# matthewyjiang/safe_bayesian_optimization

Hardware: AMD Instinct MI355X
Metric: GP posterior+acq grid-points/sec at N train pts; 1/2/4/8 GPU (higher is better)
Workload: dtype f32 (bf16x3-split MFMA, f32 accumulation)

## Files before the change

safe_bayesian_optimization_amd/csrc/diag/predict_x3_diag.hip:

```cpp
#include <cstdint>
#include <cstdlib>
#include <algorithm>
#include <type_traits>
#include <vector>

#include "../sbo_internal.hpp"

namespace sbo {
namespace {

typedef float f32x4 __attribute__((ext_vector_type(4)));
typedef float f32x2 __attribute__((ext_vector_type(2)));
typedef __bf16 bf16x2 __attribute__((ext_vector_type(2)));
typedef __bf16 bf16x8 __attribute__((ext_vector_type(8)));
typedef unsigned int u32x4 __attribute__((ext_vector_type(4)));

constexpr int kXH = 32;
constexpr int kXPlane = kBM * kXH * 2;
constexpr int kXA = 3 * kXPlane;
constexpr int kXC = 4 * kXH * 4;
constexpr int kXQ = 2 * kBN * 4;
constexpr int kXSlot = kXA + kXC + kXQ;
constexpr int kXSlots = 3;
constexpr int kXWin = kXSlots * kXSlot;
// ... 422 lines not shown
            }                                                                                           \
            if (lane < 32) SBO_DMA16(kc3 + (uint32_t)(kcf_) + (h_) * (kXC / 4), d_ + kXA);              \
        }                                                                                               \
        const char *s_ = a_base + ((DIAG & 8) ? 0 : (uint64_t)((akib_) + (h_) * (kXA / 1024)) * 1024u);  \
        const uint32_t w_ = lds_wave + (uint32_t)(sl_) * kXSlot;                                        \
        a_src = s_;                                                                                     \
        a_dst = w_;                                                                                     \
        if (!(DIAG & 2) && is_loader && ((burst_) || !(DIAG & 16)))                                     \
            _Pragma("unroll") for (int j = 0; j < kPieces; ++j)                                         \
                SBO_DMA16(s_ + j * kLoaders * 1024, w_ + (uint32_t)(j * kLoaders * 1024));              \
    } while (0)
#define SBO_REC_WINDOW(w_)                                                                              \
    do {                                                                                                \
        if (lw == 1) SBO_DMA16(reinterpret_cast<const char *>(rec) + (uint64_t)(w_) * 1024u, lds_rwin + (uint32_t)((w_) & 1) * 1024u); \
    } while (0)
    auto rec_at = [&](uint32_t e) {
        const int4 d = rwin[((e / kRecWin) & 1) * kRecWin + e % kRecWin];
        return make_int4(__builtin_amdgcn_readfirstlane(d.x), __builtin_amdgcn_readfirstlane(d.y),
                         __builtin_amdgcn_readfirstlane(d.z), __builtin_amdgcn_readfirstlane(d.w));
    };
    uint32_t la_e, e_end;
    {
        const int4 da = desc[k0], db = desc[k1 - 1];
        la_e = (uint32_t)__builtin_amdgcn_readfirstlane(da.z);
        e_end = (uint32_t)__builtin_amdgcn_readfirstlane(db.z) + (uint32_t)(__builtin_amdgcn_readfirstlane(db.w) & 0xffff);
    }
    SBO_REC_WINDOW(la_e / kRecWin);
    SBO_REC_WINDOW(la_e / kRecWin + 1);
    asm volatile("s_waitcnt vmcnt(0)" ::: "memory");
    __syncthreads();
    int la_h = 0;

    const char *a_base = ax3 + (is_loader ? ldr : 0) * 1024;
    const char *a_src = ax3;
    uint32_t a_dst = 0;
    int4 r_cur = rec_at(la_e);
    auto stage = [&](int sl, bool burst) {
        const int4 r = r_cur;
        XStep s;
        s.I = min(r.w & 0xffff, nI - 1);
        s.qb = r.z;
        s.flags = la_h | ((r.w & kRecFirst) && la_h == 0 ? kFirst : 0) | ((r.w & kRecLast) && la_h == 1 ? kLast : 0) |
                  kValid;
        s.lv = LEVELS ? min((r.w >> 16) & 3, 2) : 0;
        SBO_X3_STAGE(min((uint32_t)r.x, a_max), r.y, la_h, r.z, sl, burst, (s.flags & kFirst) != 0);
        la_h ^= 1;
        if (la_h == 0) {
            ++la_e;
            if (la_e % kRecWin == 1) SBO_REC_WINDOW(la_e / kRecWin + 1);
            if (la_e < e_end) r_cur = rec_at(la_e);
        }
        return s;
    };

    XStep s0 = stage(0, true), s1 = {0, 0, 0, 0}, s2 = {0, 0, 0, 0};
    if (la_e < e_end) s1 = stage(1, true);
    asm volatile("s_waitcnt vmcnt(0)" ::: "memory");
    __syncthreads();

    const int qo = WIDE ? lw * 32 + (lane & 31) : lw * 16 * NC + r;
    constexpr int kCB = NC == 2 ? 2 : 1, kRB = WIDE ? 8 : 16;
    typedef std::conditional_t<WIDE, f32x16, f32x4> AccT;
    AccT acc[kCB][kRB], outer[kCB][kRB];
#pragma unroll
    for (int c = 0; c < kCB; ++c)
#pragma unroll
// ... 274 lines not shown
            const double v = (double)h[sl * kStampFields + j];
            if (j < n) out[j] += v;
            const int o = 12 + 12 * (int)(sl % 8) + j;
            if (o < n) out[o] += v;
        }
        const int o = 108 + (int)(sl / 8);
        if (o < n) out[o] += (double)h[sl * kStampFields + 5] / 8.0;
    }
    std::fill(h.begin(), h.end(), 0ull);
    return hipMemcpyToSymbol(HIP_SYMBOL(g_x3_stamps), h.data(), h.size() * sizeof(unsigned long long));
}

hipError_t launch_predict_x3(hipStream_t s, const char *ax3, const float *kc3, const int4 *desc, const int4 *rec,
                             const int *seg, int P, int n_items, int nI, const float *qx, const float *qy, int64_t m,
                             int64_t ldp, float cexp, float m0, float *part, float *mean, int variant) {
    const int64_t amax = (total_tiles(nI) - 1) * (2 * kXA / 1024);
    if (nI <= 0 || amax > 0xffffffffll) return hipErrorInvalidValue;
    const uint32_t a_max = (uint32_t)amax;
    int rot = 0;
#ifdef SBO_DIAG
    if (const char *e = getenv("SBO_XCD_ROT")) rot = std::clamp(atoi(e), 0, 7);
#endif
#define SBO_X3_LAUNCH(NC, D) \
    hipLaunchKernelGGL((predict_x3_kernel<NC, D>), dim3((unsigned)P), dim3(NC == 1 ? 512 : 256), 0, s, ax3, kc3, desc, rec, \
                       seg, P, n_items, nI, a_max, rot, qx, qy, m, ldp, cexp, m0, part, mean)
    switch (variant) {
        case 2: SBO_X3_LAUNCH(2, 16); break;
        case 9: SBO_X3_LAUNCH(1, 0); break;
        case 10: SBO_X3_LAUNCH(1, 48); break;
        case 13: SBO_X3_LAUNCH(3, 16); break;
        case 22: SBO_X3_LAUNCH(1, 16); break;
// ... 60 lines not shown
```

safe_bayesian_optimization_amd/csrc/kernels.hip:

```cpp
#include <cstdio>
#include <cstdlib>
#include <algorithm>
#include <cstring>

#include <rocprim/rocprim.hpp>

#include "sbo_internal.hpp"

namespace sbo {
namespace {

typedef float f32x16 __attribute__((ext_vector_type(16)));

__device__ __forceinline__ float fast_exp2(float v) { return __builtin_amdgcn_exp2f(v); }

constexpr int kFillCols = 8;

template <bool VEC>
__global__ __launch_bounds__(256) void rbf_fill_kernel(const float *__restrict__ xa,
                                                       const float *__restrict__ ya, int64_t ma,
                                                       const float *__restrict__ xb,
                                                       const float *__restrict__ yb, int64_t mb,
                                                       int64_t ld, float c, float sf2, float sn2,
                                                       int diag, float *__restrict__ K) {
// ... 1876 lines not shown
    const int64_t a = xseg[x], n = xseg[x + 1] - a, q = n / G, rm = n % G, c = (k - a) % G, j = (k - a) / G;
    return a + c * q + (c < rm ? c : rm) + j;
}

__global__ void plan_perm_kernel(const unsigned long long *__restrict__ scan, int64_t n_items,
                                 const int4 *__restrict__ desc, const int *__restrict__ xseg, int G,
                                 int *__restrict__ pos_of, unsigned long long *__restrict__ cnt2) {
    const int64_t nne = (int64_t)(scan[n_items - 1] >> kPlanKeyShift);
    const int64_t k = (int64_t)blockIdx.x * blockDim.x + threadIdx.x;
    if (k >= nne) return;
    const int64_t p = xcd_position(k, xseg, G);
    pos_of[k] = (int)p;
    cnt2[p] = (unsigned long long)(desc[k].w & 0xffff);
}

__device__ __forceinline__ int4 step_record(int64_t ts, int I, int qb, int te, int i, int cnt);

__global__ __launch_bounds__(256) void plan_move_kernel(const unsigned long long *__restrict__ scan, int64_t n_items,
                                                        const int4 *__restrict__ desc,
                                                        const unsigned short *__restrict__ tl,
                                                        const int *__restrict__ pos_of,
                                                        const unsigned long long *__restrict__ off2,
                                                        int4 *__restrict__ desc2, unsigned short *__restrict__ tl2,
                                                        int4 *__restrict__ rec) {
    const int64_t nne = (int64_t)(scan[n_items - 1] >> kPlanKeyShift);
    const int64_t k = (int64_t)blockIdx.x * 4 + (threadIdx.x >> 6);
    const int lane = threadIdx.x & 63;
    if (k >= nne) return;
    const int4 d = desc[k];
    const int cnt = d.w & 0xffff;
    const uint64_t off = (uint64_t)(uint32_t)d.z | ((uint64_t)((uint32_t)d.w >> 16) << 32);
    const int p = pos_of[k];
    const uint64_t o2 = off2[p];
    const int64_t ts = tile_start(d.x);
    for (int i = lane; i < cnt; i += 64) {
        const unsigned short te = tl[off + i];
        tl2[o2 + i] = te;
        if (rec) rec[o2 + i] = step_record(ts, d.x, d.y, te, i, cnt);
    }
    if (lane == 0) desc2[p] = make_int4(d.x, d.y, (int)(uint32_t)o2, cnt | (int)((o2 >> 32) << 16));
}

__device__ __forceinline__ int4 step_record(int64_t ts, int I, int qb, int te, int i, int cnt) {
    const int t = te & ((1 << kLevelShift) - 1);
    const int w = I | ((te >> kLevelShift) << 16) | (i == 0 ? kRecFirst : 0) | (i == cnt - 1 ? kRecLast : 0);
    return make_int4((int)(uint32_t)((ts + t) * 96), t * 256, qb, w);
}

__global__ __launch_bounds__(256) void plan_rec_kernel(const unsigned long long *__restrict__ scan, int64_t n_items,
                                                       const int4 *__restrict__ desc,
                                                       const unsigned short *__restrict__ tl, int4 *__restrict__ rec) {
    const int64_t nne = (int64_t)(scan[n_items - 1] >> kPlanKeyShift);
    const int64_t k = (int64_t)blockIdx.x * 4 + (threadIdx.x >> 6);
    const int lane = threadIdx.x & 63;
    if (k >= nne) return;
    const int4 d = desc[k];
    const int cnt = d.w & 0xffff;
    const uint64_t off = (uint64_t)(uint32_t)d.z | ((uint64_t)((uint32_t)d.w >> 16) << 32);
    const int64_t ts = tile_start(d.x);
    for (int i = lane; i < cnt; i += 64) rec[off + i] = step_record(ts, d.x, d.y, tl[off + i], i, cnt);
}

__global__ void plan_seg2_kernel(const int *__restrict__ xseg, int G, int P, int *__restrict__ seg2) {
    for (int r = threadIdx.x; r <= P; r += blockDim.x) {
        if (r == P) {
            seg2[P] = xseg[8];
            continue;
        }
        const int x = r / G, c = r % G;
        const int a = xseg[x], n = xseg[x + 1] - a, q = n / G, rm = n % G;
        seg2[r] = a + c * q + (c < rm ? c : rm);
    }
}

__global__ void plan_block_cost_kernel(const unsigned long long *__restrict__ wkey, int nI, int64_t nQ,
// ... 534 lines not shown
    auto take = [&](size_t b) {
        const size_t at = o;
        o = (o + b + 255) / 256 * 256;
        return at;
    };
    L.key = take(8 * (size_t)items);
    L.scan = take(8 * (size_t)items);
    L.thr = take((size_t)items);
    L.wkey = take(8 * (size_t)items);
    L.wscan = take(8 * (size_t)items);
    L.lvcnt = take(8 * 3 * 4 * (size_t)kPlanWriteBlocks);
    L.bits = take(8 * 3 * (size_t)items * (size_t)plan_chunks((int)nI));
    L.desc = take(16 * (size_t)(items + 2 * kDescWindow));
    L.tl = take(2 * (size_t)(cap + 2 * kListWindow));
    L.seg = take(4 * (size_t)(P + 1));
    L.rec = take(16 * (size_t)(cap + 2 * kRecWindow));
    size_t tb = 0;
    (void)rocprim::inclusive_scan(nullptr, tb, (const unsigned long long *)nullptr, (unsigned long long *)nullptr,
                                  (size_t)items, rocprim::plus<unsigned long long>());
    L.temp = take(tb);
    L.temp_bytes = tb;
    L.xcd = xcd_interleave(P);
    if (L.xcd) {
        L.xseg = take(4 * 9);
        L.pos_of = take(4 * (size_t)items);
        L.cnt2 = take(8 * (size_t)items);
        L.off2 = take(8 * (size_t)items);
        L.desc2 = take(16 * (size_t)(items + 2 * kDescWindow));
        L.tl2 = take(2 * (size_t)(cap + 2 * kListWindow));
        L.seg2 = take(4 * (size_t)(P + 1));
        size_t t2 = 0;
// ... 12 lines not shown

size_t predict_work_bytes(int64_t npad, int64_t m, int P) {
    return plan_layout(npad / kBM, (m + kBN - 1) / kBN, P).total;
}

hipError_t launch_plan(hipStream_t s, const float4 *kbox, int64_t npad, const float *qx, const float *qy, int64_t m,
                       int64_t ldp, float ell, float m0, const SkipPlan &skip, float *part, float *mean,
                       unsigned long long *tiles_done, int P, void *work, size_t work_bytes) {
    const int nI = (int)(npad / kBM);
    const int64_t nQ = (m + kBN - 1) / kBN;
    const int64_t items = (int64_t)nI * nQ;
    if (m <= 0 || nI <= 0) return hipSuccess;
    if (nQ > 0x7fffffff || items >= (1ll << (64 - kPlanKeyShift)) ||
        2 * (int64_t)nI * (nI + 1) * nQ >= (1ll << kPlanKeyShift) || kTilesPerRowBlockStep * (int64_t)nI > (1 << kLevelShift) - 1)
        return hipErrorInvalidValue;
    const PlanLayout L = plan_layout(nI, nQ, P);
    if (work_bytes < L.total) return hipErrorInvalidValue;
    if (skip.order_blk != 0 && ((skip.order_blk >> 8) < 1 || (skip.order_blk & 255) < 1 || (skip.order_blk >> 16) != 0))
        return hipErrorInvalidValue;
    char *w = static_cast<char *>(work);
    auto *key = reinterpret_cast<unsigned long long *>(w + L.key);
    auto *scan = reinterpret_cast<unsigned long long *>(w + L.scan);
    auto *thr = reinterpret_cast<unsigned char *>(w + L.thr);
    auto *desc = reinterpret_cast<int4 *>(w + L.desc);
    auto *tl = reinterpret_cast<unsigned short *>(w + L.tl);
    auto *seg = reinterpret_cast<int *>(w + L.seg);
    auto *wkey = reinterpret_cast<unsigned long long *>(w + L.wkey);
    auto *wscan = reinterpret_cast<unsigned long long *>(w + L.wscan);
#ifdef SBO_DIAG
    if (const char *ev = getenv("SBO_MEAN_W")) {
// ... 29 lines not shown
    e = rocprim::inclusive_scan(w + L.temp, tb, wkey, wscan, (size_t)items, rocprim::plus<unsigned long long>(), s);
    if (e != hipSuccess) return e;
    const int64_t wblocks = std::min<int64_t>((items + 3) / 4, kPlanWriteBlocks);
    hipLaunchKernelGGL(plan_write_kernel, dim3((unsigned)wblocks), dim3(256), 0, s, nI, nQ, key, scan, bits,
                       desc, tl, skip.prod_full, tiles_done ? reinterpret_cast<unsigned long long *>(w + L.lvcnt) : nullptr,
                       skip.order_blk);
    if (tiles_done)
        hipLaunchKernelGGL(plan_counts_reduce_kernel, dim3(1), dim3(256), 0, s,
                           reinterpret_cast<const unsigned long long *>(w + L.lvcnt), wblocks * 4, tiles_done + 1);
    auto *rec = reinterpret_cast<int4 *>(w + L.rec);
    if (!L.xcd) {
        hipLaunchKernelGGL(plan_seg_kernel, dim3(1), dim3(256), 0, s, scan, items, desc, P, seg, tiles_done, wkey,
                           wscan, nI, nQ, skip.order_blk);
        if (skip.records)
            hipLaunchKernelGGL(plan_rec_kernel, dim3((unsigned)((items + 3) / 4)), dim3(256), 0, s, scan, items, desc,
                               tl, rec);
        return hipGetLastError();
    }
    auto *xseg = reinterpret_cast<int *>(w + L.xseg);
    auto *pos_of = reinterpret_cast<int *>(w + L.pos_of);
    auto *cnt2 = reinterpret_cast<unsigned long long *>(w + L.cnt2);
    auto *off2 = reinterpret_cast<unsigned long long *>(w + L.off2);
    auto *desc2 = reinterpret_cast<int4 *>(w + L.desc2);
    auto *tl2 = reinterpret_cast<unsigned short *>(w + L.tl2);
    auto *seg2 = reinterpret_cast<int *>(w + L.seg2);
    const int G = P / 8;
    e = hipMemsetAsync(cnt2, 0, 8 * (size_t)items, s);
    if (e != hipSuccess) return e;
    hipLaunchKernelGGL(plan_seg_kernel, dim3(1), dim3(256), 0, s, scan, items, desc, 8, xseg, tiles_done, wkey, wscan,
                       nI, nQ, skip.order_blk);
    hipLaunchKernelGGL(plan_perm_kernel, dim3((unsigned)((items + 255) / 256)), dim3(256), 0, s, scan, items, desc,
                       xseg, G, pos_of, cnt2);
    e = hipGetLastError();
    if (e != hipSuccess) return e;
    size_t t2 = L.temp2_bytes;
    e = rocprim::exclusive_scan(w + L.temp2, t2, cnt2, off2, 0ull, (size_t)items,
                                rocprim::plus<unsigned long long>(), s);
    if (e != hipSuccess) return e;
    hipLaunchKernelGGL(plan_move_kernel, dim3((unsigned)((items + 3) / 4)), dim3(256), 0, s, scan, items, desc, tl,
                       pos_of, off2, desc2, tl2, skip.records ? rec : nullptr);
    hipLaunchKernelGGL(plan_seg2_kernel, dim3(1), dim3(256), 0, s, xseg, G, P, seg2);
    return hipGetLastError();
}

void plan_views(int64_t npad, int64_t m, int P, const void *work, const int4 **desc, const unsigned short **tl,
                const int **seg, const int4 **rec) {
    const PlanLayout L = plan_layout(npad / kBM, (m + kBN - 1) / kBN, P);
    const char *w = static_cast<const char *>(work);
    *desc = reinterpret_cast<const int4 *>(w + (L.xcd ? L.desc2 : L.desc));
    *tl = reinterpret_cast<const unsigned short *>(w + (L.xcd ? L.tl2 : L.tl));
    *seg = reinterpret_cast<const int *>(w + (L.xcd ? L.seg2 : L.seg));
    if (rec) *rec = reinterpret_cast<const int4 *>(w + L.rec);
}

float exp2_coef_f(float ell) { return (float)exp2_coef(ell); }
// ... 82 lines not shown
```

safe_bayesian_optimization_amd/csrc/predict_x3.hip:

```cpp
#include <cstdint>
#include <vector>

#include "sbo_internal.hpp"

namespace sbo {
namespace {

typedef float f32x4 __attribute__((ext_vector_type(4)));
typedef float f32x2 __attribute__((ext_vector_type(2)));
typedef __bf16 bf16x2 __attribute__((ext_vector_type(2)));
typedef __bf16 bf16x8 __attribute__((ext_vector_type(8)));
typedef unsigned int u32x4 __attribute__((ext_vector_type(4)));

constexpr int kXH = 32;
constexpr int kXPlane = kBM * kXH * 2;
constexpr int kXA = 3 * kXPlane;
constexpr int kXC = 4 * kXH * 4;
constexpr int kXQ = 2 * kBN * 4;
constexpr int kXSlot = kXA + kXC + kXQ;
constexpr int kXSlots = 3;
constexpr int kXWin = kXSlots * kXSlot;
constexpr int kXSmem = kXWin + 4096;
constexpr int kRecWin = 64;
constexpr int kLoaders = 8;
// ... 16 lines not shown
    w1 = pk_bf16(ra, rb);
    w2 = pk_bf16(ra - lo_f32(w1), rb - hi_f32(w1));
}

__device__ __forceinline__ bf16x8 as_bf16x8(u32x4 v) { return __builtin_bit_cast(bf16x8, v); }

__device__ __forceinline__ f32x4 mfma(u32x4 a, u32x4 b, f32x4 c) {
    return __builtin_amdgcn_mfma_f32_16x16x32_bf16(as_bf16x8(a), as_bf16x8(b), c, 0, 0, 0);
}

typedef __attribute__((address_space(3))) char lds_char;

__device__ __forceinline__ u32x4 lds_b128(const lds_char *p) {
    return *reinterpret_cast<const __attribute__((address_space(3))) u32x4 *>(p);
}
__device__ __forceinline__ float lds_f(const lds_char *p) {
    return *reinterpret_cast<const __attribute__((address_space(3))) float *>(p);
}
typedef float f32x2v __attribute__((ext_vector_type(2)));
__device__ __forceinline__ f32x2v lds_f2(const lds_char *p) {
    return *reinterpret_cast<const __attribute__((address_space(3))) f32x2v *>(p);
}

__device__ __forceinline__ void dma16_masked(uint32_t voff, const void *sbase, uint32_t ldst, uint64_t mask) {
    uint64_t sv;
    asm volatile("s_mov_b64 %0, exec\n\ts_and_b64 exec, exec, %4\n\ts_nop 0\n\tglobal_load_lds_dwordx4 %1, %2\n\t"
                 "s_mov_b64 exec, %0"
                 : "=&s"(sv)
                 : "v"(voff), "s"(sbase), "{m0}"(ldst), "s"(mask)
                 : "memory", "scc");
}

struct KPieces {
    u32x4 h, m, l;
};

__device__ __forceinline__ float kstar1(float xk, float yk, float xq, float yq, float cexp) {
    const float dx = xk - xq, dy = yk - yq;
    return fast_exp2(fmaf(dy, dy, dx * dx) * cexp);
}

#define SBO_PIN(v) asm volatile("" : "+v"(v))

template <bool FRESH, int LV, bool KHN>
__device__ __forceinline__ void x3_half(const lds_char *pa, const lds_char *pcn, float xq, float yq, int g,
                                        float cexp, float msc, const KPieces &kb, f32x4 (&acc)[16],
                                        f32x4 (&outer)[16], KPieces &nx, double &mu, uint32_t voff, const char *asrc,
                                        uint32_t adst, int npieces) {
    const f32x4 zero = {0.f, 0.f, 0.f, 0.f};
    constexpr bool P1 = LV <= 1, P2 = LV == 0;
    constexpr int NPROD = LV == 0 ? 6 : (LV == 1 ? 3 : 1);
    constexpr int LAG = LV == 0 ? 2 : (LV == 1 ? 4 : 8);
    constexpr int AH = LV == 2 ? 4 : (LV == 1 ? 2 : 1);
    u32x4 f0[16], f1[16], f2[16];
#pragma unroll
    for (int r = 0; r < AH; ++r) {
        f0[r] = lds_b128(pa + r * 1024);
        if constexpr (P1) f1[r] = lds_b128(pa + kXPlane + r * 1024);
        if constexpr (P2) f2[r] = lds_b128(pa + 2 * kXPlane + r * 1024);
    }
    f32x2v xk = lds_f2(pcn + g * 32), yk = lds_f2(pcn + 128 + g * 32), ak = {0.f, 0.f};
    if (msc != 0.0f) ak = lds_f2(pcn + 256 + g * 32);
    f32x2v e;
#pragma unroll
    for (int rb = 0; rb < 16; ++rb) {
        if (rb + AH < 16) {
            f0[rb + AH] = lds_b128(pa + (rb + AH) * 1024);
            if constexpr (P1) f1[rb + AH] = lds_b128(pa + kXPlane + (rb + AH) * 1024);
            if constexpr (P2) f2[rb + AH] = lds_b128(pa + 2 * kXPlane + (rb + AH) * 1024);
        }
        const u32x4 a0 = f0[rb];
        u32x4 a1 = {}, a2 = {};
        if constexpr (P1) a1 = f1[rb];
        if constexpr (P2) a2 = f2[rb];
        const int i = rb >> 2, ph = rb & 3;
        if (ph <= 1) {
            float ev = kstar1(ph == 0 ? xk.x : xk.y, ph == 0 ? yk.x : yk.y, xq, yq, cexp);
            SBO_PIN(ev);
            if (ph == 0) e.x = ev; else e.y = ev;
            if (ph == 1 && i < 3) {
// ... 11 lines not shown
                SBO_PIN(w0);
                SBO_PIN(w1);
                SBO_PIN(w2);
                nx.h[i] = w0;
                nx.m[i] = w1;
                nx.l[i] = w2;
            }
        } else {
            if (msc != 0.0f) {
                mu += (double)fmaf(ak.x, e.x, ak.y * e.y);
                SBO_PIN(mu);
            }
            if (i < 3 && msc != 0.0f) ak = lds_f2(pcn + 256 + g * 32 + (i + 1) * 8);
        }
        if (rb >= 1 && rb <= kPieces) {
            const uint32_t mh = (uint32_t)__builtin_amdgcn_readfirstlane(rb <= npieces ? -1 : 0);
            dma16_masked(voff, asrc + (rb - 1) * kStride, adst + (rb - 1) * kStride, ((uint64_t)mh << 32) | mh);
        }
        if (!FRESH && rb >= LAG) outer[rb - LAG] += acc[rb - LAG];
        f32x4 v = FRESH ? zero : acc[rb];
        if constexpr (P2) {
            v = mfma(a2, kb.h, v);
            v = mfma(a1, kb.m, v);
            v = mfma(a0, kb.l, v);
        }
        if constexpr (P1) {
            v = mfma(a1, kb.h, v);
            v = mfma(a0, kb.m, v);
        }
        v = mfma(a0, kb.h, v);
        acc[rb] = v;
#pragma unroll
        for (int j = 0; j < NPROD; ++j) {
            __builtin_amdgcn_sched_group_barrier(0x008, 1, 0);
            __builtin_amdgcn_sched_group_barrier(0x002, 2, 0);
            __builtin_amdgcn_sched_group_barrier(0x100, 1, 0);
        }
        __builtin_amdgcn_sched_barrier(0);
    }
    if (!FRESH) {
#pragma unroll
        for (int rb = 16 - LAG; rb < 16; ++rb) outer[rb] += acc[rb];
    }
}

__device__ __forceinline__ void x3_kstar(const lds_char *pc, float xq, float yq, int g, float cexp, bool mean,
                                         KPieces &kb, double &mu) {
#pragma unroll
    for (int i = 0; i < 4; ++i) {
        const f32x2v xk = lds_f2(pc + g * 32 + i * 8), yk = lds_f2(pc + 128 + g * 32 + i * 8);
        const f32x2v ak = lds_f2(pc + 256 + g * 32 + i * 8);
        const float e0 = kstar1(xk.x, yk.x, xq, yq, cexp), e1 = kstar1(xk.y, yk.y, xq, yq, cexp);
        uint32_t w0, w1, w2;
        split3(e0, e1, w0, w1, w2);
        kb.h[i] = w0;
        kb.m[i] = w1;
        kb.l[i] = w2;
        if (mean) mu += (double)fmaf(ak.x, e0, ak.y * e1);
    }
}

struct XStep {
    int I, qb, flags;
    int lv;
};
constexpr int kFirst = 2, kLast = 4, kValid = 8;

__global__ __launch_bounds__(512, 1) void predict_x3_kernel(
    const char *__restrict__ ax3, const float *__restrict__ kc3, const int4 *__restrict__ desc,
    const int4 *__restrict__ rec, const int *__restrict__ seg, int P, int n_items, int nI, uint32_t a_max,
    const float *__restrict__ qx, const float *__restrict__ qy, int64_t m, int64_t ldp, float cexp, float m0,
    float *__restrict__ part, float *__restrict__ mean) {
    __shared__ __attribute__((aligned(16))) char smem[kXSmem];
    const int bid = blockIdx.x;
    const int rng = (P % 8 == 0) ? (bid % 8) * (P / 8) + bid / 8 : bid;
    const int k0 = max(seg[rng], 0), k1 = min(seg[rng + 1], n_items);
    if (k0 >= k1) return;
    const int tid = threadIdx.x, lane = tid & 63;
    const int lw = __builtin_amdgcn_readfirstlane(tid >> 6);
    const int g = lane >> 4, r = lane & 15;

    const lds_char *lds = (const lds_char *)smem;
    const int4 *rwin = reinterpret_cast<const int4 *>(smem + kXWin);
    const uint32_t voff = (uint32_t)lane * 16u;
    const uint32_t lds_smem = (uint32_t)(uintptr_t)(lds_char *)(smem);
    const uint32_t lds_wave = lds_smem + (uint32_t)lw * 1024u;
    const uint32_t lds_rwin = lds_smem + (uint32_t)kXWin;
#define SBO_DMA16(sbase, ldst)                                                                          \
    asm volatile("s_nop 0\n\tglobal_load_lds_dwordx4 %0, %1" ::"v"(voff), "s"((const void *)(sbase)),     \
                 "{m0}"(ldst)                                                                           \
                 : "memory")
#define SBO_X3_STAGE(akib_, kcf_, h_, qb_, sl_, burst_, first_)                                         \
    do {                                                                                                \
        const uint32_t d_ = lds_smem + (uint32_t)(sl_) * kXSlot;                                        \
        if (lw == 0) {                                                                                  \
            if (first_) {                                                                               \
                if (lane < 32) SBO_DMA16(qx + (int64_t)(qb_) * kBN, d_ + kXA + kXC);                    \
                else SBO_DMA16(qy + (int64_t)(qb_) * kBN - 128, d_ + kXA + kXC);                        \
            }                                                                                           \
            if (lane < 32) SBO_DMA16(kc3 + (uint32_t)(kcf_) + (h_) * (kXC / 4), d_ + kXA);              \
        }                                                                                               \
        const char *s_ = a_base + (uint64_t)((akib_) + (h_) * (kXA / 1024)) * 1024u;                     \
        const uint32_t w_ = lds_wave + (uint32_t)(sl_) * kXSlot;                                        \
        a_src = s_;                                                                                     \
        a_dst = w_;                                                                                     \
        if (burst_)                                                                                     \
            _Pragma("unroll") for (int j = 0; j < kPieces; ++j)                                         \
                SBO_DMA16(s_ + j * kStride, w_ + (uint32_t)(j * kStride));                              \
    } while (0)
#define SBO_REC_WINDOW(w_)                                                                              \
    do {                                                                                                \
        if (lw == 1) SBO_DMA16(reinterpret_cast<const char *>(rec) + (uint64_t)(w_) * 1024u, lds_rwin + (uint32_t)((w_) & 1) * 1024u); \
    } while (0)
    auto rec_at = [&](uint32_t e) {
        const int4 d = rwin[((e / kRecWin) & 1) * kRecWin + e % kRecWin];
        return make_int4(__builtin_amdgcn_readfirstlane(d.x), __builtin_amdgcn_readfirstlane(d.y),
                         __builtin_amdgcn_readfirstlane(d.z), __builtin_amdgcn_readfirstlane(d.w));
    };
    uint32_t la_e, e_end;
    {
        const int4 da = desc[k0], db = desc[k1 - 1];
        la_e = (uint32_t)__builtin_amdgcn_readfirstlane(da.z);
        e_end = (uint32_t)__builtin_amdgcn_readfirstlane(db.z) + (uint32_t)(__builtin_amdgcn_readfirstlane(db.w) & 0xffff);
    }
    SBO_REC_WINDOW(la_e / kRecWin);
    SBO_REC_WINDOW(la_e / kRecWin + 1);
    asm volatile("s_waitcnt vmcnt(0)" ::: "memory");
    __syncthreads();
    int la_h = 0;

    const char *a_base = ax3 + lw * 1024;
    const char *a_src = ax3;
    uint32_t a_dst = 0;
    int4 r_cur = rec_at(la_e);
    auto stage = [&](int sl, bool burst) {
        const int4 rr = r_cur;
        XStep s;
        s.I = min(rr.w & 0xffff, nI - 1);
        s.qb = rr.z;
        s.flags = la_h | ((rr.w & kRecFirst) && la_h == 0 ? kFirst : 0) | ((rr.w & kRecLast) && la_h == 1 ? kLast : 0) |
                  kValid;
        s.lv = min((rr.w >> 16) & 3, 2);
        SBO_X3_STAGE(min((uint32_t)rr.x, a_max), rr.y, la_h, rr.z, sl, burst, (s.flags & kFirst) != 0);
        la_h ^= 1;
        if (la_h == 0) {
            ++la_e;
            if (la_e % kRecWin == 1) SBO_REC_WINDOW(la_e / kRecWin + 1);
            if (la_e < e_end) r_cur = rec_at(la_e);
        }
        return s;
    };

    XStep s0 = stage(0, true), s1 = {0, 0, 0, 0}, s2 = {0, 0, 0, 0};
    if (la_e < e_end) s1 = stage(1, true);
    asm volatile("s_waitcnt vmcnt(0)" ::: "memory");
    __syncthreads();

    const int qo = lw * 16 + r;
    f32x4 acc[16], outer[16];
#pragma unroll
    for (int rb = 0; rb < 16; ++rb) {
        acc[rb] = f32x4{};
        outer[rb] = acc[rb];
    }
    double mu = 0.0;
    KPieces kb, nx;
    float xq, yq;
    {
        const lds_char *pq = lds + kXA + kXC;
        xq = lds_f(pq + qo * 4);
        yq = lds_f(pq + (kBN + qo) * 4);
        x3_kstar(lds + kXA, xq, yq, g, cexp, s0.I == nI - 1, kb, mu);
    }
    bool pend = false, pend_mean = false;
    float pend_s = 0.0f, pend_mu = 0.0f;
    int64_t pend_q = 0;
    int pend_I = 0;
    auto flush = [&]() {
        if (pend && lane < 16 && pend_q < m) {
            part[(int64_t)pend_I * ldp + pend_q] = pend_s;
            if (pend_mean) mean[pend_q] = pend_mu;
        }
        pend = false;
    };
    int cur = 0;
    bool more = true;
    auto half_step = [&](auto fresh_tag) {
        constexpr bool FRESH = decltype(fresh_tag)::value;
        if (FRESH) flush();
        const bool issue = la_e < e_end;
        const int nslot = cur == 0 ? 2 : cur - 1;
        s2 = issue ? stage(nslot, false) : XStep{0, 0, 0, 0};
        const int np2 = (kPieces / 3) * (3 - s2.lv);
        if (!issue) a_dst = lds_wave + (uint32_t)nslot * kXSlot;
        const int cslot = cur == 2 ? 0 : cur + 1;
        const lds_char *pa = lds + cur * kXSlot + lane * 16;
        const lds_char *pcn = lds + cslot * kXSlot + kXA;
        const lds_char *pqn = pcn + kXC;
        const bool nvalid = (s1.flags & kValid) != 0;
        const float msc = nvalid && s1.I == nI - 1 ? 1.0f : 0.0f;
        if (!FRESH) {
            if ((s0.flags & kLast) && s0.I == nI - 1) {
                double u = mu;
                u += __shfl_xor(u, 16);
                u += __shfl_xor(u, 32);
                pend_mu = (float)((double)m0 + u);
            }
            if (nvalid && (s1.flags & kFirst)) mu = 0.0;
        }
        if (nvalid && (s1.flags & kFirst)) {
            xq = lds_f(pqn + qo * 4);
            yq = lds_f(pqn + (kBN + qo) * 4);
        }
        if (s0.lv == 2 && nvalid && s1.lv == 2)
            x3_half<FRESH, 2, true>(pa, pcn, xq, yq, g, cexp, msc, kb, acc, outer, nx, mu, voff, a_src, a_dst, np2);
        else if (s0.lv == 2)
            x3_half<FRESH, 2, false>(pa, pcn, xq, yq, g, cexp, msc, kb, acc, outer, nx, mu, voff, a_src, a_dst, np2);
        else if (s0.lv == 1)
            x3_half<FRESH, 1, false>(pa, pcn, xq, yq, g, cexp, msc, kb, acc, outer, nx, mu, voff, a_src, a_dst, np2);
        else
            x3_half<FRESH, 0, false>(pa, pcn, xq, yq, g, cexp, msc, kb, acc, outer, nx, mu, voff, a_src, a_dst, np2);
        if (!FRESH && (s0.flags & kLast)) {
            pend = true;
            pend_I = s0.I;
            pend_q = (int64_t)s0.qb * kBN + qo;
            pend_mean = s0.I == nI - 1;
            double sq[4] = {};
#pragma unroll
            for (int rb = 0; rb < 16; ++rb)
#pragma unroll
                for (int e = 0; e < 4; ++e) {
                    sq[e] = fma((double)outer[rb][e], (double)outer[rb][e], sq[e]);
                    outer[rb][e] = 0.0f;
                }
            double sv = (sq[0] + sq[1]) + (sq[2] + sq[3]);
            sv += __shfl_xor(sv, 16);
            sv += __shfl_xor(sv, 32);
            pend_s = (float)sv;
        }
        asm volatile("s_waitcnt vmcnt(6)" ::: "memory");
        asm volatile("s_waitcnt lgkmcnt(0)\n\ts_barrier" ::: "memory");
        more = nvalid;
        s0 = s1;
        s1 = s2;
        kb = nx;
        cur = cslot;
    };
    do {
        half_step(std::integral_constant<bool, true>{});
        half_step(std::integral_constant<bool, false>{});
    } while (more);
    asm volatile("s_waitcnt vmcnt(0)" ::: "memory");
    flush();
#undef SBO_X3_STAGE
#undef SBO_REC_WINDOW
#undef SBO_DMA16
}

__global__ __launch_bounds__(256) void pack_x3_kernel(const float *__restrict__ aug, int64_t T0, int64_t nt,
                                                      char *__restrict__ ax3) {
    const int64_t id = (int64_t)blockIdx.x * 256 + threadIdx.x;
// ... 46 lines not shown
    }
    if (!kc3) return hipSuccess;
    const int64_t nkt = npad / kBK;
    hipLaunchKernelGGL(pack_kc3_kernel, dim3((unsigned)((nkt * 256 + 255) / 256)), dim3(256), 0, s, kcoord, nkt, kc3);
    return hipGetLastError();
}

hipError_t read_x3_stamps(double *out, int n) {
    for (int j = 0; j < n; ++j) out[j] = 0.0;
    return hipSuccess;
}

hipError_t launch_predict_x3(hipStream_t s, const char *ax3, const float *kc3, const int4 *desc, const int4 *rec,
                             const int *seg, int P, int n_items, int nI, const float *qx, const float *qy, int64_t m,
                             int64_t ldp, float cexp, float m0, float *part, float *mean, int variant) {
    const int64_t amax = (total_tiles(nI) - 1) * (2 * kXA / 1024);
    if (nI <= 0 || amax > 0xffffffffll) return hipErrorInvalidValue;
    if (variant != 3 && variant != 22) return hipErrorInvalidValue;
    hipLaunchKernelGGL(predict_x3_kernel, dim3((unsigned)P), dim3(512), 0, s, ax3, kc3, desc, rec, seg, P, n_items, nI,
                       (uint32_t)amax, qx, qy, m, ldp, cexp, m0, part, mean);
    return hipGetLastError();
}

}
```

safe_bayesian_optimization_amd/csrc/sbo_internal.hpp:

```cpp
#pragma once

#include <hip/hip_runtime.h>
#include <rocblas/rocblas.h>

#include <cstddef>
#include <cstdint>
#include <string>
#include <utility>
#include <vector>

#include "../../include/sbo.h"

namespace sbo {

constexpr int kBM = 256;
constexpr int kBN = 128;
constexpr int kBK = 64;
constexpr int kTileFloats = kBM * kBK;
constexpr int kTilesPerRowBlockStep = kBM / kBK;
constexpr int kAcqThreads = 256;
constexpr int64_t kMaxGridY = 65535;

__host__ __device__ inline int64_t round_up(int64_t v, int64_t m) { return (v + m - 1) / m * m; }

// ... 223 lines not shown
                       int64_t ldp, float ell, float m0, const SkipPlan &skip, float *part, float *mean,
                       unsigned long long *tiles_done, int P, void *work, size_t work_bytes);
hipError_t launch_predict(hipStream_t s, const float *aug, const float *kcoord, int64_t npad, const float *qx,
                          const float *qy, int64_t m, int64_t ldp, float ell, float m0, float *part, float *mean,
                          int variant, int P, const void *work);
float exp2_coef_f(float ell);
hipError_t launch_plan_cost(hipStream_t s, int64_t npad, int64_t m, int P, const void *work, const int32_t *perm,
                            float *bcost, float *cost);
void plan_views(int64_t npad, int64_t m, int P, const void *work, const int4 **desc, const unsigned short **tl,
                const int **seg, const int4 **rec = nullptr);
size_t x3_operand_bytes(int64_t npad);
size_t x3_coord_bytes(int64_t npad);
hipError_t launch_pack_x3(hipStream_t s, const float *aug, const float *kcoord, int64_t npad, int64_t I0, int wide,
                          char *ax3, float *kc3);
constexpr int kLevelShift = 14;
constexpr int kRecFirst = 1 << 20, kRecLast = 1 << 21;
inline bool x3_levels(int variant) { return variant == 3 || variant == 23 || variant == 24 || variant == 30 || variant == 32 || variant == 33 || variant == 39 || variant == 41 || variant == 42 || variant == 43 || variant == 46 || variant == 47 || variant == 48 || variant == 49 || variant == 51 || variant == 52 || variant == 53 || variant == 54 || variant == 55 || variant == 56 || variant == 57 || (variant >= 58 && variant <= 61); }
inline bool variant_allowed(int v) {
#ifdef SBO_DIAG
    return v >= 0 && v <= 61;
#else
    return v == 0 || v == 1 || v == 3 || v == 22;
#endif
}
inline int x3_layout(int variant) { return (variant == 13 || variant == 14) ? 1 : 0; }
hipError_t read_x3_stamps(double *out, int n);
hipError_t launch_predict_x3(hipStream_t s, const char *ax3, const float *kc3, const int4 *desc, const int4 *rec,
                             const int *seg, int P, int n_items, int nI, const float *qx, const float *qy, int64_t m,
                             int64_t ldp, float cexp, float m0, float *part, float *mean, int variant);
hipError_t launch_tile_norms(hipStream_t s, const float *aug, int64_t npad, int64_t I0, float4 *lgn);
hipError_t launch_pack_tile_norms(hipStream_t s, const double *Linv, int64_t ld, int64_t n, int64_t npad, int64_t I0,
// ... 110 lines not shown
```

Baseline: 42.83 million.

## Precompute per-half step records to cut scalar bookkeeping in x3 predict loop

The plan kernels now emit two records per step, one per half, with clamped row block, level, half, first/last, mean and piece-count flags and final addresses all precomputed. The predict loop just reads the next record from LDS, prefetched inside x3_half with a volatile load and readfirstlane, and rotates slot offsets instead of recomputing slot indices. This removes per-half scalar ALU work (mins, flag composition, branches) and hides the record read latency behind MFMA work. In exchange the record buffer doubles and the plan gains an extra size limit. It also adds optional register pinning of the outer accumulators and an s_cselect-based DMA mask.

```diff
diff --git a/safe_bayesian_optimization_amd/csrc/diag/predict_x3_diag.hip b/safe_bayesian_optimization_amd/csrc/diag/predict_x3_diag.hip
--- a/safe_bayesian_optimization_amd/csrc/diag/predict_x3_diag.hip
+++ b/safe_bayesian_optimization_amd/csrc/diag/predict_x3_diag.hip
@@ -460,8 +460,8 @@
     do {                                                                                                \
         if (lw == 1) SBO_DMA16(reinterpret_cast<const char *>(rec) + (uint64_t)(w_) * 1024u, lds_rwin + (uint32_t)((w_) & 1) * 1024u); \
     } while (0)
-    auto rec_at = [&](uint32_t e) {
-        const int4 d = rwin[((e / kRecWin) & 1) * kRecWin + e % kRecWin];
+    auto rec_at = [&](uint32_t j) {
+        const int4 d = rwin[j % (2 * kRecWin)];
         return make_int4(__builtin_amdgcn_readfirstlane(d.x), __builtin_amdgcn_readfirstlane(d.y),
                          __builtin_amdgcn_readfirstlane(d.z), __builtin_amdgcn_readfirstlane(d.w));
     };
@@ -471,8 +471,8 @@
         la_e = (uint32_t)__builtin_amdgcn_readfirstlane(da.z);
         e_end = (uint32_t)__builtin_amdgcn_readfirstlane(db.z) + (uint32_t)(__builtin_amdgcn_readfirstlane(db.w) & 0xffff);
     }
-    SBO_REC_WINDOW(la_e / kRecWin);
-    SBO_REC_WINDOW(la_e / kRecWin + 1);
+    SBO_REC_WINDOW(2 * la_e / kRecWin);
+    SBO_REC_WINDOW(2 * la_e / kRecWin + 1);
     asm volatile("s_waitcnt vmcnt(0)" ::: "memory");
     __syncthreads();
     int la_h = 0;
@@ -480,22 +480,20 @@
     const char *a_base = ax3 + (is_loader ? ldr : 0) * 1024;
     const char *a_src = ax3;
     uint32_t a_dst = 0;
-    int4 r_cur = rec_at(la_e);
+    int4 r_cur = rec_at(2 * la_e);
     auto stage = [&](int sl, bool burst) {
         const int4 r = r_cur;
         XStep s;
-        s.I = min(r.w & 0xffff, nI - 1);
+        s.I = r.w & 0xffff;
         s.qb = r.z;
-        s.flags = la_h | ((r.w & kRecFirst) && la_h == 0 ? kFirst : 0) | ((r.w & kRecLast) && la_h == 1 ? kLast : 0) |
-                  kValid;
-        s.lv = LEVELS ? min((r.w >> 16) & 3, 2) : 0;
-        SBO_X3_STAGE(min((uint32_t)r.x, a_max), r.y, la_h, r.z, sl, burst, (s.flags & kFirst) != 0);
+        s.flags = ((r.w & kRecHalf) ? 1 : 0) | ((r.w & kRecFirst) ? kFirst : 0) | ((r.w & kRecLast) ? kLast : 0) | kValid;
+        s.lv = LEVELS ? (r.w >> kRecLevelShift) & 3 : 0;
+        SBO_X3_STAGE(min((uint32_t)r.x, a_max), r.y, 0, r.z, sl, burst, (s.flags & kFirst) != 0);
         la_h ^= 1;
-        if (la_h == 0) {
-            ++la_e;
-            if (la_e % kRecWin == 1) SBO_REC_WINDOW(la_e / kRecWin + 1);
-            if (la_e < e_end) r_cur = rec_at(la_e);
-        }
+        if (la_h == 0) ++la_e;
+        const uint32_t j = 2 * la_e + (uint32_t)la_h;
+        if (j % kRecWin == 2) SBO_REC_WINDOW(j / kRecWin + 1);
+        if (la_e < e_end) r_cur = rec_at(j);
         return s;
     };
 
@@ -800,7 +798,7 @@
 hipError_t launch_predict_x3(hipStream_t s, const char *ax3, const float *kc3, const int4 *desc, const int4 *rec,
                              const int *seg, int P, int n_items, int nI, const float *qx, const float *qy, int64_t m,
                              int64_t ldp, float cexp, float m0, float *part, float *mean, int variant) {
-    const int64_t amax = (total_tiles(nI) - 1) * (2 * kXA / 1024);
+    const int64_t amax = (total_tiles(nI) - 1) * (2 * kXA / 1024) + kXA / 1024;
     if (nI <= 0 || amax > 0xffffffffll) return hipErrorInvalidValue;
     const uint32_t a_max = (uint32_t)amax;
     int rot = 0;
diff --git a/safe_bayesian_optimization_amd/csrc/kernels.hip b/safe_bayesian_optimization_amd/csrc/kernels.hip
--- a/safe_bayesian_optimization_amd/csrc/kernels.hip
+++ b/safe_bayesian_optimization_amd/csrc/kernels.hip
@@ -1914,7 +1914,7 @@
     cnt2[p] = (unsigned long long)(desc[k].w & 0xffff);
 }
 
-__device__ __forceinline__ int4 step_record(int64_t ts, int I, int qb, int te, int i, int cnt);
+__device__ __forceinline__ int4 step_record(int64_t ts, int I, int qb, int te, int i, int cnt, int nI, int h);
 
 __global__ __launch_bounds__(256) void plan_move_kernel(const unsigned long long *__restrict__ scan, int64_t n_items,
                                                         const int4 *__restrict__ desc,
@@ -1922,7 +1922,7 @@
                                                         const int *__restrict__ pos_of,
                                                         const unsigned long long *__restrict__ off2,
                                                         int4 *__restrict__ desc2, unsigned short *__restrict__ tl2,
-                                                        int4 *__restrict__ rec) {
+                                                        int4 *__restrict__ rec, int nI) {
     const int64_t nne = (int64_t)(scan[n_items - 1] >> kPlanKeyShift);
     const int64_t k = (int64_t)blockIdx.x * 4 + (threadIdx.x >> 6);
     const int lane = threadIdx.x & 63;
@@ -1936,20 +1936,30 @@
     for (int i = lane; i < cnt; i += 64) {
         const unsigned short te = tl[off + i];
         tl2[o2 + i] = te;
-        if (rec) rec[o2 + i] = step_record(ts, d.x, d.y, te, i, cnt);
+        if (rec) {
+            rec[2 * (o2 + i)] = step_record(ts, d.x, d.y, te, i, cnt, nI, 0);
+            rec[2 * (o2 + i) + 1] = step_record(ts, d.x, d.y, te, i, cnt, nI, 1);
+        }
     }
     if (lane == 0) desc2[p] = make_int4(d.x, d.y, (int)(uint32_t)o2, cnt | (int)((o2 >> 32) << 16));
 }
 
-__device__ __forceinline__ int4 step_record(int64_t ts, int I, int qb, int te, int i, int cnt) {
+__device__ __forceinline__ int4 step_record(int64_t ts, int I, int qb, int te, int i, int cnt, int nI, int h) {
     const int t = te & ((1 << kLevelShift) - 1);
-    const int w = I | ((te >> kLevelShift) << 16) | (i == 0 ? kRecFirst : 0) | (i == cnt - 1 ? kRecLast : 0);
-    return make_int4((int)(uint32_t)((ts + t) * 96), t * 256, qb, w);
+    const int lv = min((te >> kLevelShift) & 3, 2);
+    const int rb = min(I, nI - 1);
+    const int64_t tile = min(ts + t, tile_start(nI) - 1);
+    const int w = rb | (lv << kRecLevelShift) | (h ? kRecHalf : 0) | (i == 0 && h == 0 ? kRecFirst : 0) |
+                  (i == cnt - 1 && h == 1 ? kRecLast : 0) | (rb == nI - 1 ? kRecMean : 0) | kRecValid |
+                  ((2 * (3 - lv)) << kRecPiecesShift);
+    return make_int4((int)(uint32_t)(tile * (2 * kRecHalfKiB) + h * kRecHalfKiB),
+                     t * (2 * kRecHalfCoords) + h * kRecHalfCoords, qb, w);
 }
 
 __global__ __launch_bounds__(256) void plan_rec_kernel(const unsigned long long *__restrict__ scan, int64_t n_items,
                                                        const int4 *__restrict__ desc,
-                                                       const unsigned short *__restrict__ tl, int4 *__restrict__ rec) {
+                                                       const unsigned short *__restrict__ tl, int4 *__restrict__ rec,
+                                                       int nI) {
     const int64_t nne = (int64_t)(scan[n_items - 1] >> kPlanKeyShift);
     const int64_t k = (int64_t)blockIdx.x * 4 + (threadIdx.x >> 6);
     const int lane = threadIdx.x & 63;
@@ -1958,7 +1968,8 @@
     const int cnt = d.w & 0xffff;
     const uint64_t off = (uint64_t)(uint32_t)d.z | ((uint64_t)((uint32_t)d.w >> 16) << 32);
     const int64_t ts = tile_start(d.x);
-    for (int i = lane; i < cnt; i += 64) rec[off + i] = step_record(ts, d.x, d.y, tl[off + i], i, cnt);
+    for (int j = lane; j < 2 * cnt; j += 64)
+        rec[2 * off + j] = step_record(ts, d.x, d.y, tl[off + (j >> 1)], j >> 1, cnt, nI, j & 1);
 }
 
 __global__ void plan_seg2_kernel(const int *__restrict__ xseg, int G, int P, int *__restrict__ seg2) {
@@ -2523,7 +2534,7 @@
     L.desc = take(16 * (size_t)(items + 2 * kDescWindow));
     L.tl = take(2 * (size_t)(cap + 2 * kListWindow));
     L.seg = take(4 * (size_t)(P + 1));
-    L.rec = take(16 * (size_t)(cap + 2 * kRecWindow));
+    L.rec = take(16 * (size_t)(2 * cap + 2 * kRecWindow));
     size_t tb = 0;
     (void)rocprim::inclusive_scan(nullptr, tb, (const unsigned long long *)nullptr, (unsigned long long *)nullptr,
                                   (size_t)items, rocprim::plus<unsigned long long>());
@@ -2566,6 +2577,7 @@
     if (nQ > 0x7fffffff || items >= (1ll << (64 - kPlanKeyShift)) ||
         2 * (int64_t)nI * (nI + 1) * nQ >= (1ll << kPlanKeyShift) || kTilesPerRowBlockStep * (int64_t)nI > (1 << kLevelShift) - 1)
         return hipErrorInvalidValue;
+    if (skip.records && 2 * (int64_t)nI * (nI + 1) * nQ >= (1ll << 31)) return hipErrorInvalidValue;
     const PlanLayout L = plan_layout(nI, nQ, P);
     if (work_bytes < L.total) return hipErrorInvalidValue;
     if (skip.order_blk != 0 && ((skip.order_blk >> 8) < 1 || (skip.order_blk & 255) < 1 || (skip.order_blk >> 16) != 0))
@@ -2625,7 +2637,7 @@
                            wscan, nI, nQ, skip.order_blk);
         if (skip.records)
             hipLaunchKernelGGL(plan_rec_kernel, dim3((unsigned)((items + 3) / 4)), dim3(256), 0, s, scan, items, desc,
-                               tl, rec);
+                               tl, rec, nI);
         return hipGetLastError();
     }
     auto *xseg = reinterpret_cast<int *>(w + L.xseg);
@@ -2649,7 +2661,7 @@
                                 rocprim::plus<unsigned long long>(), s);
     if (e != hipSuccess) return e;
     hipLaunchKernelGGL(plan_move_kernel, dim3((unsigned)((items + 3) / 4)), dim3(256), 0, s, scan, items, desc, tl,
-                       pos_of, off2, desc2, tl2, skip.records ? rec : nullptr);
+                       pos_of, off2, desc2, tl2, skip.records ? rec : nullptr, nI);
     hipLaunchKernelGGL(plan_seg2_kernel, dim3(1), dim3(256), 0, s, xseg, G, P, seg2);
     return hipGetLastError();
 }
diff --git a/safe_bayesian_optimization_amd/csrc/predict_x3.hip b/safe_bayesian_optimization_amd/csrc/predict_x3.hip
--- a/safe_bayesian_optimization_amd/csrc/predict_x3.hip
+++ b/safe_bayesian_optimization_amd/csrc/predict_x3.hip
@@ -54,6 +54,9 @@
 __device__ __forceinline__ u32x4 lds_b128(const lds_char *p) {
     return *reinterpret_cast<const __attribute__((address_space(3))) u32x4 *>(p);
 }
+__device__ __forceinline__ u32x4 lds_b128_here(const lds_char *p) {
+    return *reinterpret_cast<const volatile __attribute__((address_space(3))) u32x4 *>(p);
+}
 __device__ __forceinline__ float lds_f(const lds_char *p) {
     return *reinterpret_cast<const __attribute__((address_space(3))) float *>(p);
 }
@@ -82,11 +85,15 @@
 
 #define SBO_PIN(v) asm volatile("" : "+v"(v))
 
+#ifndef SBO_X3_OUTER_PIN
+#define SBO_X3_OUTER_PIN 7
+#endif
+
 template <bool FRESH, int LV, bool KHN>
 __device__ __forceinline__ void x3_half(const lds_char *pa, const lds_char *pcn, float xq, float yq, int g,
                                         float cexp, float msc, const KPieces &kb, f32x4 (&acc)[16],
                                         f32x4 (&outer)[16], KPieces &nx, double &mu, uint32_t voff, const char *asrc,
-                                        uint32_t adst, int npieces) {
+                                        uint32_t adst, int npieces, const lds_char *prec, int4 &rnx) {
     const f32x4 zero = {0.f, 0.f, 0.f, 0.f};
     constexpr bool P1 = LV <= 1, P2 = LV == 0;
     constexpr int NPROD = LV == 0 ? 6 : (LV == 1 ? 3 : 1);
@@ -102,8 +109,11 @@
     f32x2v xk = lds_f2(pcn + g * 32), yk = lds_f2(pcn + 128 + g * 32), ak = {0.f, 0.f};
     if (msc != 0.0f) ak = lds_f2(pcn + 256 + g * 32);
     f32x2v e;
+    u32x4 rraw = {};
+    const int nps = __builtin_amdgcn_readfirstlane(npieces);
 #pragma unroll
     for (int rb = 0; rb < 16; ++rb) {
+        if (rb == 16 - AH) rraw = lds_b128_here(prec);
         if (rb + AH < 16) {
             f0[rb + AH] = lds_b128(pa + (rb + AH) * 1024);
             if constexpr (P1) f1[rb + AH] = lds_b128(pa + kXPlane + (rb + AH) * 1024);
@@ -145,10 +155,14 @@
             if (i < 3 && msc != 0.0f) ak = lds_f2(pcn + 256 + g * 32 + (i + 1) * 8);
         }
         if (rb >= 1 && rb <= kPieces) {
-            const uint32_t mh = (uint32_t)__builtin_amdgcn_readfirstlane(rb <= npieces ? -1 : 0);
-            dma16_masked(voff, asrc + (rb - 1) * kStride, adst + (rb - 1) * kStride, ((uint64_t)mh << 32) | mh);
-        }
-        if (!FRESH && rb >= LAG) outer[rb - LAG] += acc[rb - LAG];
+            uint64_t mask;
+            asm("s_cmp_ge_u32 %1, %2\n\ts_cselect_b64 %0, -1, 0" : "=s"(mask) : "s"(nps), "n"(rb) : "scc");
+            dma16_masked(voff, asrc + (rb - 1) * kStride, adst + (rb - 1) * kStride, mask);
+        }
+        if (!FRESH && rb >= LAG) {
+            outer[rb - LAG] += acc[rb - LAG];
+            if constexpr (((SBO_X3_OUTER_PIN) >> LV) & 1) SBO_PIN(outer[rb - LAG]);
+        }
         f32x4 v = FRESH ? zero : acc[rb];
         if constexpr (P2) {
             v = mfma(a2, kb.h, v);
@@ -169,6 +183,11 @@
         }
         __builtin_amdgcn_sched_barrier(0);
     }
+    rnx.x = __builtin_amdgcn_readfirstlane((int)rraw.x);
+    rnx.y = __builtin_amdgcn_readfirstlane((int)rraw.y);
+    rnx.z = __builtin_amdgcn_readfirstlane((int)rraw.z);
+    rnx.w = __builtin_amdgcn_readfirstlane((int)rraw.w);
+    asm volatile("" : "+s"(rnx.x), "+s"(rnx.y), "+s"(rnx.z), "+s"(rnx.w));
     if (!FRESH) {
 #pragma unroll
         for (int rb = 16 - LAG; rb < 16; ++rb) outer[rb] += acc[rb];
@@ -195,7 +214,7 @@
     int I, qb, flags;
     int lv;
 };
-constexpr int kFirst = 2, kLast = 4, kValid = 8;
+constexpr int kFirst = kRecFirst, kLast = kRecLast, kValid = kRecValid;
 
 __global__ __launch_bounds__(512, 1) void predict_x3_kernel(
     const char *__restrict__ ax3, const float *__restrict__ kc3, const int4 *__restrict__ desc,
@@ -221,18 +240,18 @@
     asm volatile("s_nop 0\n\tglobal_load_lds_dwordx4 %0, %1" ::"v"(voff), "s"((const void *)(sbase)),     \
                  "{m0}"(ldst)                                                                           \
                  : "memory")
-#define SBO_X3_STAGE(akib_, kcf_, h_, qb_, sl_, burst_, first_)                                         \
+#define SBO_X3_STAGE(akib_, kcf_, qb_, sl_, burst_, first_)                                             \
     do {                                                                                                \
-        const uint32_t d_ = lds_smem + (uint32_t)(sl_) * kXSlot;                                        \
+        const uint32_t d_ = lds_smem + (uint32_t)(sl_);                                                 \
         if (lw == 0) {                                                                                  \
             if (first_) {                                                                               \
                 if (lane < 32) SBO_DMA16(qx + (int64_t)(qb_) * kBN, d_ + kXA + kXC);                    \
                 else SBO_DMA16(qy + (int64_t)(qb_) * kBN - 128, d_ + kXA + kXC);                        \
             }                                                                                           \
-            if (lane < 32) SBO_DMA16(kc3 + (uint32_t)(kcf_) + (h_) * (kXC / 4), d_ + kXA);              \
+            if (lane < 32) SBO_DMA16(kc3 + (uint32_t)(kcf_), d_ + kXA);                                 \
         }                                                                                               \
-        const char *s_ = a_base + (uint64_t)((akib_) + (h_) * (kXA / 1024)) * 1024u;                     \
-        const uint32_t w_ = lds_wave + (uint32_t)(sl_) * kXSlot;                                        \
+        const char *s_ = a_base + (uint64_t)(akib_) * 1024u;                                            \
+        const uint32_t w_ = lds_wave + (uint32_t)(sl_);                                                 \
         a_src = s_;                                                                                     \
         a_dst = w_;                                                                                     \
         if (burst_)                                                                                     \
@@ -244,46 +263,44 @@
         if (lw == 1) SBO_DMA16(reinterpret_cast<const char *>(rec) + (uint64_t)(w_) * 1024u, lds_rwin + (uint32_t)((w_) & 1) * 1024u); \
     } while (0)
     auto rec_at = [&](uint32_t e) {
-        const int4 d = rwin[((e / kRecWin) & 1) * kRecWin + e % kRecWin];
+        const int4 d = rwin[e % (2 * kRecWin)];
         return make_int4(__builtin_amdgcn_readfirstlane(d.x), __builtin_amdgcn_readfirstlane(d.y),
                          __builtin_amdgcn_readfirstlane(d.z), __builtin_amdgcn_readfirstlane(d.w));
     };
     uint32_t la_e, e_end;
     {
         const int4 da = desc[k0], db = desc[k1 - 1];
-        la_e = (uint32_t)__builtin_amdgcn_readfirstlane(da.z);
-        e_end = (uint32_t)__builtin_amdgcn_readfirstlane(db.z) + (uint32_t)(__builtin_amdgcn_readfirstlane(db.w) & 0xffff);
+        la_e = 2u * (uint32_t)__builtin_amdgcn_readfirstlane(da.z);
+        e_end = 2u * ((uint32_t)__builtin_amdgcn_readfirstlane(db.z) + (uint32_t)(__builtin_amdgcn_readfirstlane(db.w) & 0xffff));
     }
     SBO_REC_WINDOW(la_e / kRecWin);
     SBO_REC_WINDOW(la_e / kRecWin + 1);
     asm volatile("s_waitcnt vmcnt(0)" ::: "memory");
     __syncthreads();
-    int la_h = 0;
 
     const char *a_base = ax3 + lw * 1024;
     const char *a_src = ax3;
     uint32_t a_dst = 0;
     int4 r_cur = rec_at(la_e);
-    auto stage = [&](int sl, bool burst) {
+    auto stage = [&](uint32_t sl, bool burst) {
         const int4 rr = r_cur;
         XStep s;
-        s.I = min(rr.w & 0xffff, nI - 1);
+        s.I = rr.w & 0xffff;
         s.qb = rr.z;
-        s.flags = la_h | ((rr.w & kRecFirst) && la_h == 0 ? kFirst : 0) | ((rr.w & kRecLast) && la_h == 1 ? kLast : 0) |
-                  kValid;
-        s.lv = min((rr.w >> 16) & 3, 2);
-        SBO_X3_STAGE(min((uint32_t)rr.x, a_max), rr.y, la_h, rr.z, sl, burst, (s.flags & kFirst) != 0);
-        la_h ^= 1;
-        if (la_h == 0) {
-            ++la_e;
-            if (la_e % kRecWin == 1) SBO_REC_WINDOW(la_e / kRecWin + 1);
-            if (la_e < e_end) r_cur = rec_at(la_e);
-        }
+        s.flags = rr.w;
+        s.lv = (rr.w >> kRecLevelShift) & 3;
+        SBO_X3_STAGE(min((uint32_t)rr.x, a_max), rr.y, rr.z, sl, burst, (s.flags & kFirst) != 0);
+        ++la_e;
+        if (la_e % kRecWin == 2) SBO_REC_WINDOW(la_e / kRecWin + 1);
         return s;
     };
 
     XStep s0 = stage(0, true), s1 = {0, 0, 0, 0}, s2 = {0, 0, 0, 0};
-    if (la_e < e_end) s1 = stage(1, true);
+    r_cur = rec_at(la_e);
+    if (la_e < e_end) {
+        s1 = stage(kXSlot, true);
+        r_cur = rec_at(la_e);
+    }
     asm volatile("s_waitcnt vmcnt(0)" ::: "memory");
     __syncthreads();
 
@@ -314,28 +331,29 @@
         }
         pend = false;
     };
-    int cur = 0;
+    uint32_t o_cur = 0, o_nxt = kXSlot, o_nn = 2 * kXSlot;
     bool more = true;
     auto half_step = [&](auto fresh_tag) {
         constexpr bool FRESH = decltype(fresh_tag)::value;
         if (FRESH) flush();
         const bool issue = la_e < e_end;
-        const int nslot = cur == 0 ? 2 : cur - 1;
-        s2 = issue ? stage(nslot, false) : XStep{0, 0, 0, 0};
-        const int np2 = (kPieces / 3) * (3 - s2.lv);
-        if (!issue) a_dst = lds_wave + (uint32_t)nslot * kXSlot;
-        const int cslot = cur == 2 ? 0 : cur + 1;
-        const lds_char *pa = lds + cur * kXSlot + lane * 16;
-        const lds_char *pcn = lds + cslot * kXSlot + kXA;
+        s2 = issue ? stage(o_nn, false) : XStep{0, 0, 0, 0};
+        const int np2 = (s2.flags >> kRecPiecesShift) & 7;
+        if (!issue) a_dst = lds_wave + o_nn;
+        const lds_char *prec = lds + kXWin + (la_e % (2 * kRecWin)) * 16;
+        const lds_char *pa = lds + o_cur + lane * 16;
+        const lds_char *pcn = lds + o_nxt + kXA;
         const lds_char *pqn = pcn + kXC;
         const bool nvalid = (s1.flags & kValid) != 0;
-        const float msc = nvalid && s1.I == nI - 1 ? 1.0f : 0.0f;
+        const float msc = (s1.flags & kRecMean) ? 1.0f : 0.0f;
         if (!FRESH) {
             if ((s0.flags & kLast) && s0.I == nI - 1) {
                 double u = mu;
                 u += __shfl_xor(u, 16);
                 u += __shfl_xor(u, 32);
-                pend_mu = (float)((double)m0 + u);
+                float m0s = m0;
+                asm volatile("" : "+s"(m0s));
+                pend_mu = (float)((double)m0s + u);
             }
             if (nvalid && (s1.flags & kFirst)) mu = 0.0;
         }
@@ -344,13 +362,13 @@
             yq = lds_f(pqn + (kBN + qo) * 4);
         }
         if (s0.lv == 2 && nvalid && s1.lv == 2)
-            x3_half<FRESH, 2, true>(pa, pcn, xq, yq, g, cexp, msc, kb, acc, outer, nx, mu, voff, a_src, a_dst, np2);
+            x3_half<FRESH, 2, true>(pa, pcn, xq, yq, g, cexp, msc, kb, acc, outer, nx, mu, voff, a_src, a_dst, np2, prec, r_cur);
         else if (s0.lv == 2)
-            x3_half<FRESH, 2, false>(pa, pcn, xq, yq, g, cexp, msc, kb, acc, outer, nx, mu, voff, a_src, a_dst, np2);
+            x3_half<FRESH, 2, false>(pa, pcn, xq, yq, g, cexp, msc, kb, acc, outer, nx, mu, voff, a_src, a_dst, np2, prec, r_cur);
         else if (s0.lv == 1)
-            x3_half<FRESH, 1, false>(pa, pcn, xq, yq, g, cexp, msc, kb, acc, outer, nx, mu, voff, a_src, a_dst, np2);
+            x3_half<FRESH, 1, false>(pa, pcn, xq, yq, g, cexp, msc, kb, acc, outer, nx, mu, voff, a_src, a_dst, np2, prec, r_cur);
         else
-            x3_half<FRESH, 0, false>(pa, pcn, xq, yq, g, cexp, msc, kb, acc, outer, nx, mu, voff, a_src, a_dst, np2);
+            x3_half<FRESH, 0, false>(pa, pcn, xq, yq, g, cexp, msc, kb, acc, outer, nx, mu, voff, a_src, a_dst, np2, prec, r_cur);
         if (!FRESH && (s0.flags & kLast)) {
             pend = true;
             pend_I = s0.I;
@@ -375,7 +393,10 @@
         s0 = s1;
         s1 = s2;
         kb = nx;
-        cur = cslot;
+        const uint32_t o_free = o_cur;
+        o_cur = o_nxt;
+        o_nxt = o_nn;
+        o_nn = o_free;
     };
     do {
         half_step(std::integral_constant<bool, true>{});
@@ -452,7 +473,7 @@
 hipError_t launch_predict_x3(hipStream_t s, const char *ax3, const float *kc3, const int4 *desc, const int4 *rec,
                              const int *seg, int P, int n_items, int nI, const float *qx, const float *qy, int64_t m,
                              int64_t ldp, float cexp, float m0, float *part, float *mean, int variant) {
-    const int64_t amax = (total_tiles(nI) - 1) * (2 * kXA / 1024);
+    const int64_t amax = (total_tiles(nI) - 1) * (2 * kXA / 1024) + kXA / 1024;
     if (nI <= 0 || amax > 0xffffffffll) return hipErrorInvalidValue;
     if (variant != 3 && variant != 22) return hipErrorInvalidValue;
     hipLaunchKernelGGL(predict_x3_kernel, dim3((unsigned)P), dim3(512), 0, s, ax3, kc3, desc, rec, seg, P, n_items, nI,
diff --git a/safe_bayesian_optimization_amd/csrc/sbo_internal.hpp b/safe_bayesian_optimization_amd/csrc/sbo_internal.hpp
--- a/safe_bayesian_optimization_amd/csrc/sbo_internal.hpp
+++ b/safe_bayesian_optimization_amd/csrc/sbo_internal.hpp
@@ -261,7 +261,9 @@
 hipError_t launch_pack_x3(hipStream_t s, const float *aug, const float *kcoord, int64_t npad, int64_t I0, int wide,
                           char *ax3, float *kc3);
 constexpr int kLevelShift = 14;
-constexpr int kRecFirst = 1 << 20, kRecLast = 1 << 21;
+constexpr int kRecLevelShift = 16, kRecPiecesShift = 24;
+constexpr int kRecHalf = 1 << 18, kRecFirst = 1 << 19, kRecLast = 1 << 20, kRecMean = 1 << 21, kRecValid = 1 << 22;
+constexpr int kRecHalfKiB = 48, kRecHalfCoords = 128;
 inline bool x3_levels(int variant) { return variant == 3 || variant == 23 || variant == 24 || variant == 30 || variant == 32 || variant == 33 || variant == 39 || variant == 41 || variant == 42 || variant == 43 || variant == 46 || variant == 47 || variant == 48 || variant == 49 || variant == 51 || variant == 52 || variant == 53 || variant == 54 || variant == 55 || variant == 56 || variant == 57 || (variant >= 58 && variant <= 61); }
 inline bool variant_allowed(int v) {
 #ifdef SBO_DIAG
```

New measurement: 42.92 million (median of 3 runs). No clear change (+0.2%).
